# cs4247/music-transcription

Hardware: AMD Instinct MI355X
Metric: 30 s audio chunks/sec (mel+CNNRNN forward) (higher is better)
Workload: dtype f16; 1 GPU; CNNRNNModel inference, batch=32x30 s synthetic 16 kHz audio, mel+CNN-RNN HIP path (BASELINE.json configs[1]); batch_per_gpu=32, frames=938, coscheduled_batches_per_forward=4, streams_per_gpu=4, batches_in_flight=16, parallelism=dp1 (independent chunks)

## Files before the change

include/mt_hip.h:

```cpp
#ifndef MT_HIP_H
#define MT_HIP_H

#include <stddef.h>
#include <stdint.h>

#ifdef __cplusplus
extern "C" {
#endif

#define MT_OK            0
#define MT_EINVAL       -1
#define MT_EWORKSPACE   -2
#define MT_EHIP         -3
#define MT_EUNSUPPORTED -4

#define MT_DT_BF16 0
#define MT_DT_F16  1
#define MT_GX_F16  0x10

#define MT_N_FFT 2048
#define MT_N_PITCH 88

typedef void* mt_stream_t;

// ... 72 lines not shown
                              int B, int T, int N, int Hprev, mt_stream_t stream);
int    mt_gemm_f32acc_dt(const void* A, int lda, const void* W, int ldw, const float* bias,
                         float* C, int ldc, int M, int N, int K, int dt, mt_stream_t stream);
int    mt_gemm_lstm_gx_dt(const void* X, int ldx, const void* W_ih, int ldw, const float* bias, float* gx,
                          int B, int T, int H, int K, int dt, mt_stream_t stream);
int    mt_gemm_logits_dt(const void* X, int ldx, const void* W, int ldw, const float* bias, float* logits,
                         int B, int T, int N, int K, int dt, mt_stream_t stream);
#define MT_GEMM_SCHED_BYTES 64
size_t mt_gemm_sched_bytes(void);
int    mt_gemm_lstm_gx_sched(const void* X, int ldx, const void* W_ih, int ldw, const float* bias, float* gx,
                             int B, int T, int H, int K, int dt, void* sched, mt_stream_t stream);
int    mt_gemm_lstm_gx_from_hx_sched(const float* hx_prev, const void* W_ih, int ldw, const float* bias, float* gx,
                                     int B, int T, int H, int Hprev, int gx_f16, void* sched, mt_stream_t stream);

size_t mt_lstm_gx_bytes(int B, int T, int H);
size_t mt_lstm_hx_bytes(int B, int T, int H);
size_t mt_lstm_sync_bytes(int B, int H);
int    mt_lstm_bidir_fwd(const float* gx, const float* w_hh, float* hx, void* sync_ws, size_t sync_bytes,
                         int B, int T, int H, mt_stream_t stream);
int    mt_lstm_bidir_fwd_xproj(const float* hx_prev, const float* w_ihx, const float* bias, const float* w_hh, float* hx,
                               void* sync_ws, size_t sync_bytes, int B, int T, int H, mt_stream_t stream);
int    mt_lstm_bidir_fwd_ex(const float* gx, const float* w_hh, float* hx, void* sync_ws, size_t sync_bytes,
                            int B, int T, int H, int flags, mt_stream_t stream);
int    mt_persistent_cus_in_flight(mt_stream_t stream);
int    mt_lstm_relayout_bf16(const float* hx, void* X, int ldx, int B, int T, int H, mt_stream_t stream);
int    mt_lstm_unpack_f32(const float* hx, float* y, int B, int T, int H, mt_stream_t stream);

#define MT_MAX_LSTM_LAYERS 8
typedef struct {
    int n_mels;
    int hidden;
    int layers;
    int operand_dtype;
    const float* conv1_w;
    const float* conv1_b;
    const void*  conv2_w;
    const float* conv2_b;
    const void*  w_ih[MT_MAX_LSTM_LAYERS];
    const float* b_gates[MT_MAX_LSTM_LAYERS];
    const float* w_hh[MT_MAX_LSTM_LAYERS];
    const void*  fc_w;
    const float* fc_b;
    const float* w_ihx[MT_MAX_LSTM_LAYERS];
} mt_cnnrnn_weights;

size_t mt_cnnrnn_workspace_bytes(const mt_cnnrnn_weights* w, int B, int T);
// ... 301 lines not shown
```

music-transcription_amd/_lib.py:

```python
from __future__ import annotations

import ctypes as C
import os

_HERE = os.path.dirname(os.path.abspath(__file__))
LIB_PATH = os.path.join(_HERE, "libmt_hip.so")
MAX_LSTM_LAYERS = 8
N_PITCH = 88
DT_BF16, DT_F16 = 0, 1
GX_F16 = 0x10


class MtError(RuntimeError):
    pass


def build(verbose: bool = False) -> str:
    import subprocess
    r = subprocess.run(["make", "-C", os.path.join(_HERE, "csrc"), "-j8"], capture_output=True, text=True)
    if verbose or r.returncode != 0:
        print(r.stdout[-4000:], r.stderr[-4000:])
    if r.returncode != 0:
        raise MtError("building libmt_hip.so failed")
    return LIB_PATH
# ... 63 lines not shown
    "mt_conv_cl_dt": (i32, [vp, vp, vp, vp, vp] + [i32] * 12 + [vp]),
    "mt_gemm_batched_f32_dt": (i32, [vp, i32, ll, ll, vp, i32, ll, ll, vp, vp, i32, ll, ll, i32, i32, i32, i32, i32, i32, vp]),
    "mt_gemm_batched_h16out_dt": (i32, [vp, i32, ll, ll, vp, i32, ll, ll, vp, vp, i32, ll, ll, i32, i32, i32, i32, i32, i32, i32, vp]),
    "mt_lstm_relayout_dt": (i32, [vp, vp, i32, vp, i32, i32, i32, i32, i32, i32, i32, vp]),
    "mt_attn_softmax_clamped_dt": (i32, [vp, i32, vp, i32, i32, ll, C.c_float, C.c_float, i32, vp]),
    "mt_layernorm_residual_dt": (i32, [vp, i32, vp, i32, vp, vp, vp, i32, ll, i32, C.c_float, i32, vp]),
    "mt_gemm_lstm_gx_from_hx": (i32, [vp, vp, i32, vp, vp, i32, i32, i32, i32, vp]),
    "mt_gemm_lstm_gx_from_hx_ex": (i32, [vp, vp, i32, vp, vp, i32, i32, i32, i32, i32, vp]),
    "mt_gemm_logits_from_hx": (i32, [vp, vp, i32, vp, vp, i32, i32, i32, i32, vp]),
    "mt_gemm_bf16_f32acc": (i32, [vp, i32, vp, i32, vp, vp, i32, i32, i32, i32, vp]),
    "mt_gemm_lstm_gx": (i32, [vp, i32, vp, i32, vp, vp, i32, i32, i32, i32, vp]),
    "mt_gemm_sched_bytes": (sz, []),
    "mt_gemm_lstm_gx_sched": (i32, [vp, i32, vp, i32, vp, vp, i32, i32, i32, i32, i32, vp, vp]),
    "mt_gemm_lstm_gx_from_hx_sched": (i32, [vp, vp, i32, vp, vp, i32, i32, i32, i32, i32, vp, vp]),
    "mt_gemm_lstm_dh": (i32, [vp, i32, vp, i32, vp, i32, i32, i32, i32, i32, C.c_float, C.c_uint, C.c_uint, vp]),
    "mt_gemm_logits": (i32, [vp, i32, vp, i32, vp, vp, i32, i32, i32, i32, vp]),
    "mt_lstm_gx_bytes": (sz, [i32, i32, i32]),
    "mt_lstm_hx_bytes": (sz, [i32, i32, i32]),
    "mt_lstm_sync_bytes": (sz, [i32, i32]),
    "mt_lstm_bidir_fwd": (i32, [vp, vp, vp, vp, sz, i32, i32, i32, vp]),
    "mt_lstm_bidir_fwd_xproj": (i32, [vp, vp, vp, vp, vp, vp, sz, i32, i32, i32, vp]),
    "mt_lstm_bidir_fwd_ex": (i32, [vp, vp, vp, vp, sz, i32, i32, i32, i32, vp]),
    "mt_persistent_cus_in_flight": (i32, [vp]),
    "mt_lstm_relayout_bf16": (i32, [vp, vp, i32, i32, i32, i32, vp]),
    "mt_lstm_unpack_f32": (i32, [vp, vp, i32, i32, i32, vp]),
    "mt_conv_cl_bf16": (i32, [vp, vp, vp, vp, vp] + [i32] * 11 + [vp]),
    "mt_gemm_batched_f32": (i32, [vp, i32, ll, ll, vp, i32, ll, ll, vp, vp, i32, ll, ll, i32, i32, i32, i32, i32, vp]),
    "mt_gemm_batched_bf16out": (i32, [vp, i32, ll, ll, vp, i32, ll, ll, vp, vp, i32, ll, ll, i32, i32, i32, i32, i32, i32, vp]),
    "mt_lstm_relayout_ex": (i32, [vp, vp, i32, vp, i32, i32, i32, i32, i32, i32, vp]),
    "mt_attn_softmax_clamped": (i32, [vp, i32, vp, i32, i32, ll, C.c_float, C.c_float, vp]),
    "mt_attn_transpose_v": (i32, [vp, i32, i32, vp, i32, i32, i32, i32, i32, vp]),
    "mt_attn_fused_clamped": (i32, [vp, i32, i32, vp, i32, i32, i32, i32, i32, C.c_float, C.c_float, vp, i32, i32, vp]),
    "mt_layernorm_residual": (i32, [vp, i32, vp, i32, vp, vp, vp, i32, ll, i32, C.c_float, vp]),
    "mt_cnnrnn_large_workspace_bytes": (sz, [C.POINTER(CnnRnnLargeWeights), i32, i32]),
    "mt_cnnrnn_large_status_offset": (sz, [C.POINTER(CnnRnnLargeWeights), i32, i32, i32]),
    "mt_cnnrnn_large_forward": (i32, [C.POINTER(CnnRnnLargeWeights), vp, vp, i32, i32, vp, vp, sz, vp]),
    "mt_cnnrnn_large_forward_ex": (i32, [C.POINTER(CnnRnnLargeWeights), vp, vp, i32, i32, vp, vp, sz, vp, vp, vp, vp]),
    "mt_cnnrnn_large_num_stages": (i32, [i32]),
    "mt_cnnrnn_large_forward_ev": (i32, [C.POINTER(CnnRnnLargeWeights), vp, vp, i32, i32, vp, vp, sz, C.POINTER(vp), i32, vp]),
    "mt_adam_workspace_bytes": (sz, []),
    "mt_adam_clip_step": (i32, [vp, vp, vp, vp, ll] + [C.c_float] * 6 + [i32, vp, vp, sz, vp]),
    "mt_adam_clip_step_ex": (i32, [vp, vp, vp, vp, ll] + [C.c_float] * 6 + [i32, C.c_float, vp, i32, vp, vp, sz, vp]),
    "mt_adam_clip_step_ema": (i32, [vp, vp, vp, vp, vp, ll] + [C.c_float] * 6 + [i32, C.c_float, vp, i32, C.c_float, vp, vp, sz, vp]),
    "mt_swap_f32": (i32, [vp, vp, ll, vp]),
    "mt_bce_workspace_bytes": (sz, []),
    "mt_bce_masked_fwd_bwd": (i32, [vp, vp, vp, C.c_longlong, C.c_float, i32, vp, vp, vp, sz, i32, i32, i32, vp]),
# ... 109 lines not shown
```

music-transcription_amd/csrc/lstm.hip:

```cpp
#include "lstm_handoff.h"
#include <stdlib.h>

namespace mt {

struct LstmArgs {
    const float* gx;
    const float* w_hh;
    float* hx;
    unsigned* status;
    int B, T, H;
    int g0;
    int ngl;
    float* gates_out;
    float* cx;
    const float* w_ihx;
    const float* bias;
    const float* hx_prev;
    int sleep_first, sleep_retry;
};

__device__ __forceinline__ float sigmoidf_(float x) { return __builtin_amdgcn_rcpf(1.0f + __expf(-x)); }
__device__ __forceinline__ float tanhf_(float x) { return fmaf(2.0f, __builtin_amdgcn_rcpf(1.0f + __expf(-2.0f * x)), -1.0f); }
constexpr unsigned H_POISON = 0xFFFFFFFFu;
constexpr int PAYLOAD_POLL_SLEEP = 10;
constexpr int PAYLOAD_POLL_SLEEP_BUSY = 18;
constexpr int PAYLOAD_POLL_SLEEP_TRAIN = 12;

#ifdef MT_LSTM_DIAG
__device__ unsigned long long mt_lstm_diag[1024][8];
#define DIAG_STAMP(i) do { if (tid == 0) { const long long n_ = __builtin_amdgcn_s_memrealtime(); dg[i] += n_ - tl; tl = n_; } } while (0)
#else
#define DIAG_STAMP(i) do { } while (0)
#endif

typedef __attribute__((__vector_size__(4 * sizeof(int)))) int i32x4_t;
__device__ __forceinline__ i32x4_t raw_rsrc(const void* p, unsigned bytes) {
    const unsigned long long a = (unsigned long long)p;
    i32x4_t r;
    r[0] = __builtin_amdgcn_readfirstlane((int)(unsigned)a);
    r[1] = __builtin_amdgcn_readfirstlane((int)((unsigned)(a >> 32) & 0xffffu));
    r[2] = __builtin_amdgcn_readfirstlane((int)bytes);
    r[3] = 0x00020000;
    return r;
}
template <int OFF> __device__ __forceinline__ void asm_load_b128_sc1(u32x4& dst, int voff, i32x4_t rsrc) {
    asm volatile("buffer_load_dwordx4 %0, %1, %2, 0 offen offset:%3 sc1" : "=v"(dst) : "v"(voff), "s"(rsrc), "n"(OFF));
}
template <int NKSW, int I = 0> __device__ __forceinline__ void asm_gather_sc1(u32x4 (&hq)[NKSW], int voff, i32x4_t rsrc) {
    if constexpr (I < NKSW) {
        asm_load_b128_sc1<(I & 3) * 1024>(hq[I], voff + (I >> 2) * 4096, rsrc);
        asm_gather_sc1<NKSW, I + 1>(hq, voff, rsrc);
    }
}
__device__ __forceinline__ unsigned spin_clock() {
    return (unsigned)__builtin_amdgcn_readfirstlane((int)(unsigned)__builtin_amdgcn_s_memrealtime()) | 1u;
}
template <int N> __device__ __forceinline__ void vm_wait() { asm volatile("s_waitcnt vmcnt(%0)" :: "n"(N)); }
__device__ __forceinline__ void vm_settle(u32x4& v) { asm volatile("" : "+v"(v)); }

template <int NKSW, bool TRAIN = false, bool XP = false, int NG = 1, bool G16 = false>
__global__ __launch_bounds__(XP ? 256 : 320, XP ? 1 : (NKSW > 8 ? 2 : 4)) void lstm_rec_kernel(LstmArgs a) {
    __shared__ __attribute__((aligned(16))) float red[4][64][20];
    __shared__ __attribute__((aligned(16))) f16_t hs[32][8];
    constexpr int GX_RING = XP ? 1 : 6;
    constexpr int GX_DMA = G16 ? 2 : 4;
    __shared__ __attribute__((aligned(16))) float gring[GX_RING][XP ? 4 : (G16 ? 512 : 1024)];
    __shared__ int abort_s;
    const int tid = threadIdx.x, wv = __builtin_amdgcn_readfirstlane(tid >> 6), lane = tid & 63;
    const int H = a.H, T = a.T, nkb = H >> 3, nks = H >> 4;
    const int kb = blockIdx.x, d = blockIdx.y, gbase = blockIdx.z * NG + a.g0;
    const int ngh = min(NG, a.g0 + a.ngl - gbase);
    const int b = lane & 31, hh = lane >> 5;

    if (!XP && wv == 4) {
        typedef __attribute__((address_space(1))) void gvoid_t;
        typedef __attribute__((address_space(3))) void lvoid_t;
        const size_t gd_blocks_l = (size_t)T * 2 * nkb;
        const int nslots = T * ngh;
        int is = 0, ig = 0;
        auto request = [&](int n) {
            const int tn = d ? (T - 1 - is) : is;
            const size_t blk = (size_t)(gbase + ig) * gd_blocks_l + ((size_t)tn * 2 + d) * nkb + kb;
            const char* src = (const char*)a.gx + blk * (G16 ? 2048 : 4096) + lane * 16;
            char* dst = (char*)&gring[n % GX_RING][0];
#pragma unroll
            for (int qq = 0; qq < GX_DMA; ++qq) __builtin_amdgcn_global_load_lds((gvoid_t*)(src + qq * 1024), (lvoid_t*)(dst + qq * 1024), 16, 0, 0);
            if (++ig == ngh) { ig = 0; ++is; }
        };
        for (int n = 0; n < GX_RING - 1 && n < nslots; ++n) request(n);
        if (GX_RING - 1 <= nslots) asm volatile("s_waitcnt vmcnt(%0)" :: "n"(GX_DMA * (GX_RING - 2)) : "memory");
        else asm volatile("s_waitcnt vmcnt(0)" ::: "memory");
        __builtin_amdgcn_s_barrier();
        for (int n = 0; n < nslots; ++n) {
// ... 222 lines not shown
        }
#ifdef MT_LSTM_DIAG
        asm volatile("" :: "v"(hval));
#endif
        DIAG_STAMP(4);
        hs[b][jl] = (f16_t)hval;
        DIAG_STAMP(5);
        __syncthreads();
        if (wv == 0 && lane < 32) {
            const u32x4 piece = *(const u32x4*)(&hs[b][0]);
            const int hoff = ((t * 2 + d) * nkb) * 512 + (kb >> 1) * 1024 + ((kb & 1) * 32 + b) * 16;
            __builtin_amdgcn_raw_buffer_store_b128(piece, hrsrc, hoff, 0, 16 );
        }
        DIAG_STAMP(6);
      }
    }
    if (NG > 1) vm_wait<0>();
#ifdef MT_LSTM_DIAG
    if (tid == 0) {
        const int wg = (blockIdx.z * gridDim.y + blockIdx.y) * gridDim.x + blockIdx.x;
        for (int i = 0; i < 8; ++i) mt_lstm_diag[wg & 1023][i] = dg[i];
    }
#endif
}

template <int NK, bool TRAIN, bool G16>
__global__ __launch_bounds__(320, 4) void lstm_rec16_kernel(LstmArgs a) {
    __shared__ __attribute__((aligned(16))) float red[4][2][64][4];
    __shared__ __attribute__((aligned(16))) f16_t hs[32][8];
    constexpr int GX_RING = 6;
    constexpr int GX_DMA = G16 ? 2 : 4;
    __shared__ __attribute__((aligned(16))) float gring[GX_RING][G16 ? 512 : 1024];
    __shared__ int abort_s;
    const int tid = threadIdx.x, wv = tid >> 6, lane = tid & 63;
    const int H = a.H, T = a.T, nkb = H >> 3, nks = H >> 4;
    const int kb = blockIdx.x, d = blockIdx.y, g = blockIdx.z + a.g0;
    const int Bg = min(16, a.B - g * 32);
    const size_t gd_blocks = (size_t)T * 2 * nkb;

    if (wv == 4) {
        typedef __attribute__((address_space(1))) void gvoid_t;
        typedef __attribute__((address_space(3))) void lvoid_t;
        int is = 0;
        auto request = [&](int n) {
            const int tn = d ? (T - 1 - is) : is;
            const size_t blk = (size_t)g * gd_blocks + ((size_t)tn * 2 + d) * nkb + kb;
// ... 162 lines not shown
                                                         pack_bf16x2((float)h8[4], (float)h8[5]), pack_bf16x2((float)h8[6], (float)h8[7]));
            } else {
                for (int j = 0; j < 8 && kb * 8 + j < Hv; ++j) X[m * ldx + c0 + j] = f32_to_h16<DT>((float)h8[j]);
            }
        }
        if (Y)
            for (int j = 0; j < 8 && kb * 8 + j < Hv; ++j) Y[m * ldy + c0 + j] = (float)h8[j];
    }
}

__global__ void lstm_unpack_kernel(const f16_t* __restrict__ hx, float* __restrict__ y, int B, int T, int H) {
    const int nkb = H >> 3;
    const size_t total = (size_t)T * B * 2 * H;
    for (size_t id = (size_t)blockIdx.x * blockDim.x + threadIdx.x; id < total; id += (size_t)gridDim.x * blockDim.x) {
        const int k = id % H;
        const int d = (id / H) & 1;
        const size_t bt = id / (2 * H);
        const int t = bt % T, b = bt / T, g = b >> 5, bl = b & 31;
        const f16_t* blk = hx + ((((size_t)g * T + t) * 2 + d) * nkb) * 256 + (size_t)(k >> 4) * 512;
        y[id] = (float)blk[(((k >> 3) & 1) * 32 + bl) * 8 + (k & 7)];
    }
}

template <int NKSW, bool G16>
static int launch_rec_plain(const LstmArgs& a, int ngroups, hipStream_t st) {
    const dim3 one_set(a.H >> 3, 2, 1);
    if constexpr (NKSW <= 8) {
        if (ngroups == 2) return persistent_launch(lstm_rec_kernel<NKSW, false, false, 2, G16>, one_set, 320, a, st, "mt_lstm_bidir_fwd");
        if (ngroups == 3) return persistent_launch(lstm_rec_kernel<NKSW, false, false, 3, G16>, one_set, 320, a, st, "mt_lstm_bidir_fwd");
        if (ngroups > 3) return persistent_launch(lstm_rec_kernel<NKSW, false, false, 4, G16>, dim3(a.H >> 3, 2, cdiv(ngroups, 4)), 320, a, st, "mt_lstm_bidir_fwd");
    }
    return persistent_launch(lstm_rec_kernel<NKSW, false, false, 1, G16>, dim3(a.H >> 3, 2, ngroups), 320, a, st, "mt_lstm_bidir_fwd");
}

template <int NKSW>
static int launch_rec(const LstmArgs& a, int ngroups, bool g16, hipStream_t st) {
    const dim3 per_group(a.H >> 3, 2, ngroups);
    if constexpr (NKSW <= 8) {
        static const bool c16 = !(getenv("MT_LSTM_C16") && atoi(getenv("MT_LSTM_C16")) == 0);
        constexpr int NK16 = (NKSW + 1) / 2;
        if (c16 && !a.w_ihx && a.B <= 16 && ngroups == 1) {
            if (a.cx) return persistent_launch(lstm_rec16_kernel<NK16, true, false>, per_group, 320, a, st, "mt_lstm_bidir_fwd_train");
            if (g16) return persistent_launch(lstm_rec16_kernel<NK16, false, true>, per_group, 320, a, st, "mt_lstm_bidir_fwd");
            return persistent_launch(lstm_rec16_kernel<NK16, false, false>, per_group, 320, a, st, "mt_lstm_bidir_fwd");
        }
        if (a.w_ihx) return persistent_launch(lstm_rec_kernel<NKSW, false, true>, per_group, 256, a, st, "mt_lstm_bidir_fwd_xproj");
    }
    if (a.cx) return persistent_launch(lstm_rec_kernel<NKSW, true, false>, per_group, 320, a, st, "mt_lstm_bidir_fwd_train");
    return g16 ? launch_rec_plain<NKSW, true>(a, ngroups, st) : launch_rec_plain<NKSW, false>(a, ngroups, st);
}

}

using namespace mt;

extern "C" size_t mt_lstm_gx_bytes(int B, int T, int H) { return (size_t)cdiv(B, 32) * T * 2 * (H >> 3) * 4096; }
extern "C" size_t mt_lstm_hx_bytes(int B, int T, int H) { return (size_t)cdiv(B, 32) * T * 2 * (H >> 3) * 512; }
extern "C" size_t mt_lstm_sync_bytes(int B, int H) { (void)B; (void)H; return 512; }

static int lstm_fwd_impl(const float* gx, const float* w_hh, float* hx, void* sync_ws, size_t sync_bytes,
                         int B, int T, int H, int flags, mt_stream_t stream, float* cx = nullptr,
                         const float* w_ihx = nullptr, const float* bias = nullptr, const float* hx_prev = nullptr) {
    MT_REQUIRE((gx || w_ihx) && w_hh && hx && sync_ws, MT_EINVAL, "mt_lstm_bidir_fwd: null pointer");
    MT_REQUIRE(B > 0 && T > 0 && H >= 16 && H % 16 == 0 && H <= 1024, MT_EUNSUPPORTED,
               "mt_lstm_bidir_fwd: hidden size %d unsupported (multiple of 16, <= 1024)", H);
    MT_REQUIRE(sync_bytes >= mt_lstm_sync_bytes(B, H), MT_EWORKSPACE, "mt_lstm_bidir_fwd: sync workspace too small");
    const int nkb = H >> 3, ng = cdiv(B, 32);
    const bool g16 = (flags & MT_GX_F16) != 0;
    MT_REQUIRE(!g16 || (!cx && !w_ihx), MT_EINVAL, "mt_lstm_bidir_fwd_ex: MT_GX_F16 is for plain inference launches only");
    MT_REQUIRE((size_t)T * 2 * nkb * 512 < ((size_t)1 << 31), MT_EUNSUPPORTED, "mt_lstm_bidir_fwd: T*H too large for one buffer descriptor");
    MT_REQUIRE(!cx || (size_t)T * 2 * nkb * 4096 < ((size_t)1 << 31), MT_EUNSUPPORTED, "mt_lstm_bidir_fwd_train: T*H too large for one buffer descriptor of the gates");
    MT_REQUIRE((((size_t)w_hh | (size_t)w_ihx) & 15) == 0, MT_EINVAL, "mt_lstm_bidir_fwd: weight matrices must be 16-byte aligned");
    hipStream_t st = (hipStream_t)stream;
    MT_CHECK_HIP(hipMemsetAsync(sync_ws, 0, mt_lstm_sync_bytes(B, H), st));
    MT_CHECK_HIP(hipMemsetAsync(hx, 0xFF, mt_lstm_hx_bytes(B, T, H), st));
    static const int env_first = getenv("MT_LSTM_POLL_FIRST") ? atoi(getenv("MT_LSTM_POLL_FIRST")) : -1;
    static const int env_retry = getenv("MT_LSTM_POLL_RETRY") ? atoi(getenv("MT_LSTM_POLL_RETRY")) : -1;
    LstmArgs a{gx, w_hh, hx, (unsigned*)sync_ws, B, T, H, 0, 0,
               cx ? const_cast<float*>(gx) : nullptr, cx, w_ihx, bias, hx_prev,
               env_first >= 0 ? env_first : (cx ? PAYLOAD_POLL_SLEEP_TRAIN : ((!w_ihx && mt_persistent_cus_in_flight(stream) > 0) ? PAYLOAD_POLL_SLEEP_BUSY : PAYLOAD_POLL_SLEEP)),
               env_retry >= 0 ? env_retry : 0};
    const int zmax = (256 / (2 * nkb)) > 0 ? (256 / (2 * nkb)) : 1;
    const int nksw = cdiv(nkb / 2, 4);
    const int per_launch = (cx || w_ihx || nksw > 8) ? zmax : 4 * zmax;
    for (int g0 = 0; g0 < ng; g0 += per_launch) {
        a.g0 = g0;
        const int n = (ng - g0) < per_launch ? (ng - g0) : per_launch;
        a.ngl = n;
        int rc;
        if (nksw <= 1) rc = launch_rec<1>(a, n, g16, st);
        else if (nksw <= 2) rc = launch_rec<2>(a, n, g16, st);
        else if (nksw <= 4) rc = launch_rec<4>(a, n, g16, st);
        else if (nksw <= 8) rc = launch_rec<8>(a, n, g16, st);
        else rc = launch_rec<16>(a, n, g16, st);
        if (rc != MT_OK) return rc;
    }
    return MT_OK;
}

extern "C" int mt_lstm_bidir_fwd(const float* gx, const float* w_hh, float* hx, void* sync_ws, size_t sync_bytes,
                                 int B, int T, int H, mt_stream_t stream) {
    return lstm_fwd_impl(gx, w_hh, hx, sync_ws, sync_bytes, B, T, H, 0, stream);
}

extern "C" int mt_lstm_bidir_fwd_xproj(const float* hx_prev, const float* w_ihx, const float* bias, const float* w_hh, float* hx,
                                       void* sync_ws, size_t sync_bytes, int B, int T, int H, mt_stream_t stream) {
    MT_REQUIRE(hx_prev && w_ihx && bias && hx_prev != hx, MT_EINVAL, "mt_lstm_bidir_fwd_xproj: bad arguments");
    MT_REQUIRE(H <= 512, MT_EUNSUPPORTED, "mt_lstm_bidir_fwd_xproj: H=%d > 512 (the W_ih slice lives in registers)", H);
    return lstm_fwd_impl(nullptr, w_hh, hx, sync_ws, sync_bytes, B, T, H, 0, stream, nullptr, w_ihx, bias, hx_prev);
}

extern "C" int mt_lstm_bidir_fwd_train(float* gx_inout, const float* w_hh, float* hx, float* cx, void* sync_ws, size_t sync_bytes,
                                       int B, int T, int H, mt_stream_t stream) {
    MT_REQUIRE(cx, MT_EINVAL, "mt_lstm_bidir_fwd_train: null cx");
    return lstm_fwd_impl(gx_inout, w_hh, hx, sync_ws, sync_bytes, B, T, H, 0, stream, cx);
}

extern "C" int mt_lstm_bidir_fwd_ex(const float* gx, const float* w_hh, float* hx, void* sync_ws, size_t sync_bytes,
                                    int B, int T, int H, int flags, mt_stream_t stream) {
    MT_REQUIRE(flags == 0 || flags == MT_GX_F16, MT_EINVAL, "mt_lstm_bidir_fwd_ex: flags must be 0 or MT_GX_F16 (gx is f16)");
    return lstm_fwd_impl(gx, w_hh, hx, sync_ws, sync_bytes, B, T, H, flags, stream);
}

extern "C" int mt_lstm_relayout_dt(const float* hx, void* X, int ldx, float* Y, int ldy, int col_off, int B, int T, int H, int Hv,
                                   int dt, mt_stream_t stream) {
    MT_REQUIRE(hx && (X || Y) && H % 16 == 0 && Hv > 0 && Hv <= H && col_off >= 0, MT_EINVAL, "mt_lstm_relayout_ex: bad arguments");
    MT_REQUIRE((!X || (ldx >= col_off + 2 * Hv && ldx % 8 == 0)) && (!Y || ldy >= col_off + 2 * Hv), MT_EINVAL, "mt_lstm_relayout_ex: bad leading dimension");
    MT_REQUIRE_DT(dt, "mt_lstm_relayout");
    const size_t total = (size_t)T * B * 2 * ((Hv + 7) >> 3);
    MT_REQUIRE(total < ((size_t)1 << 31), MT_EUNSUPPORTED, "mt_lstm_relayout: more than 2^31 pieces");
    const int blocks = (int)((total + 255) / 256 < 4096 ? (total + 255) / 256 : 4096);
    const Div3 dv = make_div3((Hv + 7) >> 3, 2);
    unsigned mB, sB;
    div_magic((unsigned)B, &mB, &sB);
    if (dt == MT_DT_F16)
        hipLaunchKernelGGL(lstm_relayout_kernel<MT_DT_F16>, dim3(blocks), dim3(256), 0, (hipStream_t)stream, (const f16_t*)hx, (bf16_t*)X, ldx, Y, ldy,
                           col_off, B, T, H, Hv, dv, mB, sB);
    else
        hipLaunchKernelGGL(lstm_relayout_kernel<MT_DT_BF16>, dim3(blocks), dim3(256), 0, (hipStream_t)stream, (const f16_t*)hx, (bf16_t*)X, ldx, Y, ldy,
                           col_off, B, T, H, Hv, dv, mB, sB);
    MT_CHECK_LAUNCH();
    return MT_OK;
}
extern "C" int mt_lstm_relayout_ex(const float* hx, void* X, int ldx, float* Y, int ldy, int col_off, int B, int T, int H, int Hv,
                                   mt_stream_t stream) {
// ... 23 lines not shown
```

music-transcription_amd/csrc/lstm_handoff.h:

```cpp
#pragma once
#include "mt_common.h"

namespace mt {

constexpr int LSTM_SPIN_LIMIT_TICKS = 200000000;
constexpr int OOB_OFF = 0x7FFFFF00;
typedef __attribute__((__vector_size__(4 * sizeof(unsigned)))) unsigned u32x4;

__device__ __forceinline__ void sleep64(int n) {
    for (int i = 0; i < n; ++i) __builtin_amdgcn_s_sleep(1);
}

int persistent_admit(const void* kernel, int block, size_t smem, int nwg, hipStream_t st, const char* who);
int persistent_mark(hipStream_t st);
int persistent_cancel(hipStream_t st);

template <typename Args>
static int persistent_launch(void (*kernel)(Args), dim3 grid, int nthreads, const Args& a, hipStream_t st, const char* who,
                             const char* file = __builtin_FILE(), int line = __builtin_LINE()) {
    int rc = persistent_admit((const void*)kernel, nthreads, 0, (int)(grid.x * grid.y * grid.z), st, who);
    if (rc != MT_OK) return rc;
    hipLaunchKernelGGL(kernel, grid, dim3(nthreads), 0, st, a);
    const hipError_t e = hipGetLastError();
    if (e != hipSuccess) {
        persistent_cancel(st);
        set_error("%s:%d: persistent launch -> %s", file, line, hipGetErrorString(e));
        return MT_EHIP;
    }
    return persistent_mark(st);
}

}
```

music-transcription_amd/csrc/model.hip:

```cpp
#include "mt_common.h"
#include <stdlib.h>

extern "C" {
int mt_conv1_bn_relu_pool_dt(const float*, const float*, const float*, const float*, void*, int, int, int, int, mt_stream_t);
int mt_conv2_bn_relu_pool_dt(const void*, const void*, const float*, void*, int, int, int, int, int, mt_stream_t);
int mt_conv12_bn_relu_pool_dt(const float*, const float*, const float*, const float*, const void*, const float*, void*, int, int, int, int, int, mt_stream_t);
int mt_gemm_lstm_gx_dt(const void*, int, const void*, int, const float*, float*, int, int, int, int, int, mt_stream_t);
int mt_gemm_logits_dt(const void*, int, const void*, int, const float*, float*, int, int, int, int, int, mt_stream_t);
int mt_lstm_bidir_fwd_ex(const float*, const float*, float*, void*, size_t, int, int, int, int, mt_stream_t);
int mt_lstm_relayout_dt(const float*, void*, int, float*, int, int, int, int, int, int, int, mt_stream_t);
int mt_gemm_lstm_gx_from_hx_ex(const float*, const void*, int, const float*, float*, int, int, int, int, int, mt_stream_t);
int mt_gemm_logits_from_hx(const float*, const void*, int, const float*, float*, int, int, int, int, mt_stream_t);
int mt_gemm_lstm_gx_sched(const void*, int, const void*, int, const float*, float*, int, int, int, int, int, void*, mt_stream_t);
int mt_gemm_lstm_gx_from_hx_sched(const float*, const void*, int, const float*, float*, int, int, int, int, int, void*, mt_stream_t);
int mt_lstm_bidir_fwd_xproj(const float*, const float*, const float*, const float*, float*, void*, size_t, int, int, int, mt_stream_t);
size_t mt_lstm_gx_bytes(int, int, int);
size_t mt_lstm_hx_bytes(int, int, int);
size_t mt_lstm_sync_bytes(int, int);
}

namespace mt {
struct CnnRnnPlan {
    int F1, Fo2, K0, K1, M, Mpad, Hp;
    size_t act1, x0, x1, gx, hx, hx2, sync, sync_stride, sched, total;
// ... 68 lines not shown
    MT_REQUIRE(B > 0 && T > 0, MT_EINVAL, "mt_cnnrnn_forward: bad dims B=%d T=%d", B, T);
    const CnnRnnPlan p = plan(w, B, T);
    MT_REQUIRE(workspace_bytes >= p.total, MT_EWORKSPACE, "mt_cnnrnn_forward: workspace %zu < %zu bytes", workspace_bytes, p.total);
    char* ws = (char*)workspace;
    const int H = p.Hp, Hv = w->hidden, dt = w->operand_dtype;
    hipStream_t st = (hipStream_t)stream;
    int ei = 0;
    if ((rc = rec(events, n_events, ei, st)) != MT_OK) return rc;
    if (mt_cnnrnn_conv_fused()) {
        if ((rc = rec(events, n_events, ei, st)) != MT_OK) return rc;
        if ((rc = mt_conv12_bn_relu_pool_dt(mel, chunk_max_power, w->conv1_w, w->conv1_b, w->conv2_w, w->conv2_b, ws + p.x0, p.K0, B, w->n_mels, T, dt,
                                            stream)) != MT_OK) return rc;
    } else {
        if ((rc = mt_conv1_bn_relu_pool_dt(mel, chunk_max_power, w->conv1_w, w->conv1_b, ws + p.act1, B, w->n_mels, T, dt, stream)) != MT_OK) return rc;
        if ((rc = rec(events, n_events, ei, st)) != MT_OK) return rc;
        if ((rc = mt_conv2_bn_relu_pool_dt(ws + p.act1, w->conv2_w, w->conv2_b, ws + p.x0, p.K0, B, p.F1, T, dt, stream)) != MT_OK) return rc;
    }
    if ((rc = rec(events, n_events, ei, st)) != MT_OK) return rc;
    if (p.K1 != 2 * Hv) MT_CHECK_HIP(hipMemsetAsync(ws + p.x1, 0, (size_t)p.Mpad * p.K1 * 2, (hipStream_t)stream));
    char* hcur = ws + p.hx;
    char* hnext = ws + p.hx2;
    const bool from_hx = dt == MT_DT_F16 && H == Hv && H % 64 == 0;
    const int gx16 = (dt == MT_DT_F16) ? MT_GX_F16 : 0;
    for (int l = 0; l < w->layers; ++l) {
        const bool last = l + 1 == w->layers;
        const bool fused = l > 0 && w->w_ihx[l] && H <= 512;
        if (fused) {
            if ((rc = rec(events, n_events, ei, st)) != MT_OK) return rc;
            if ((rc = mt_lstm_bidir_fwd_xproj((const float*)hcur, w->w_ihx[l], w->b_gates[l], w->w_hh[l], (float*)hnext,
                                              ws + p.sync + p.sync_stride * l, p.sync_stride, B, T, H, stream)) != MT_OK) return rc;
            char* tmp = hcur; hcur = hnext; hnext = tmp;
        } else {
            const int K = l == 0 ? p.K0 : p.K1;
            if (l > 0 && from_hx) {
                if ((rc = mt_gemm_lstm_gx_from_hx_sched((const float*)hcur, w->w_ih[l], K, w->b_gates[l], (float*)(ws + p.gx), B, T, H, H, gx16,
                                                        ws + p.sched + (size_t)MT_GEMM_SCHED_BYTES * l, stream)) != MT_OK) return rc;
                char* tmp = hcur; hcur = hnext; hnext = tmp;
            } else {
                const void* X = l == 0 ? ws + p.x0 : ws + p.x1;
                if ((rc = mt_gemm_lstm_gx_sched(X, K, w->w_ih[l], K, w->b_gates[l], (float*)(ws + p.gx), B, T, H, K, dt | gx16,
                                                ws + p.sched + (size_t)MT_GEMM_SCHED_BYTES * l, stream)) != MT_OK) return rc;
            }
            if ((rc = rec(events, n_events, ei, st)) != MT_OK) return rc;
            if ((rc = mt_lstm_bidir_fwd_ex((const float*)(ws + p.gx), w->w_hh[l], (float*)hcur, ws + p.sync + p.sync_stride * l,
                                           p.sync_stride, B, T, H, gx16, stream)) != MT_OK) return rc;
        }
        if ((rc = rec(events, n_events, ei, st)) != MT_OK) return rc;
        const bool next_fused = !last && w->w_ihx[l + 1] && H <= 512;
        if (!next_fused && !from_hx)
            if ((rc = mt_lstm_relayout_dt((const float*)hcur, ws + p.x1, p.K1, nullptr, 0, 0, B, T, H, Hv, dt, stream)) != MT_OK) return rc;
        if ((rc = rec(events, n_events, ei, st)) != MT_OK) return rc;
    }
    if (from_hx) {
        if ((rc = mt_gemm_logits_from_hx((const float*)hcur, w->fc_w, p.K1, w->fc_b, logits, B, T, MT_N_PITCH, H, stream)) != MT_OK) return rc;
    } else {
        if ((rc = mt_gemm_logits_dt(ws + p.x1, p.K1, w->fc_w, p.K1, w->fc_b, logits, B, T, MT_N_PITCH, p.K1, dt, stream)) != MT_OK) return rc;
    }
    return rec(events, n_events, ei, st);
}

extern "C" int mt_cnnrnn_forward(const mt_cnnrnn_weights* w, const float* mel, const float* chunk_max_power, int B, int T,
                                 float* logits, void* workspace, size_t workspace_bytes, mt_stream_t stream) {
    return mt_cnnrnn_forward_ex(w, mel, chunk_max_power, B, T, logits, workspace, workspace_bytes, nullptr, 0, stream);
}
```

music-transcription_amd/csrc/residency.hip:

```cpp
#include "mt_common.h"
#include <mutex>
#include <vector>

namespace mt {

struct PersistentEntry {
    hipStream_t st;
    hipEvent_t ev;
    double need;
    bool pending;
    int reserved;
    double rneed;
};
static std::mutex g_mu;
static std::vector<PersistentEntry> g_tab[16];
static int g_ncu[16];

int persistent_admit(const void* kernel, int block, size_t smem, int nwg, hipStream_t st, const char* who) {
    int dev = 0;
    MT_CHECK_HIP(hipGetDevice(&dev));
    MT_REQUIRE(dev >= 0 && dev < 16, MT_EUNSUPPORTED, "%s: device index %d", who, dev);
    int per_cu = 0;
    MT_CHECK_HIP(hipOccupancyMaxActiveBlocksPerMultiprocessor(&per_cu, kernel, block, smem));
    MT_REQUIRE(per_cu >= 1, MT_EUNSUPPORTED, "%s: the kernel does not fit a CU", who);
    std::lock_guard<std::mutex> lock(g_mu);
    if (g_ncu[dev] == 0) MT_CHECK_HIP(hipDeviceGetAttribute(&g_ncu[dev], hipDeviceAttributeMultiprocessorCount, dev));
    const double need = (double)nwg / per_cu, cap = (double)g_ncu[dev];
    MT_REQUIRE(need <= cap, MT_EUNSUPPORTED, "%s: %d workgroups at %d per CU cannot be resident on %d CUs", who, nwg, per_cu, g_ncu[dev]);
    double others = 0.0;
    PersistentEntry* mine = nullptr;
    for (auto& e : g_tab[dev]) {
        if (e.pending && hipEventQuery(e.ev) == hipSuccess) { e.pending = false; e.need = 0.0; }
        if (e.st == st) mine = &e;
        else others += (e.pending ? e.need : 0.0) > e.rneed ? (e.pending ? e.need : 0.0) : e.rneed;
    }
    (void)hipGetLastError();
    if (others + need > cap + 1e-9) {
        set_error("%s: %.0f CUs for this persistent launch + %.0f CUs held by persistent launches pending on other streams > %d CUs: "
                  "they could not all be resident and would stall on each other (fewer forwards in flight per GPU)",
                  who, need, others, g_ncu[dev]);
        return MT_EUNSUPPORTED;
    }
    if (!mine) {
        PersistentEntry e{st, nullptr, 0.0, false, 0, 0.0};
        MT_CHECK_HIP(hipEventCreateWithFlags(&e.ev, hipEventDisableTiming));
        g_tab[dev].push_back(e);
        mine = &g_tab[dev].back();
    }
    mine->reserved += 1;
    mine->rneed = mine->rneed > need ? mine->rneed : need;
    return MT_OK;
}

static PersistentEntry* find_entry(int dev, hipStream_t st) {
    for (auto& e : g_tab[dev])
        if (e.st == st) return &e;
    return nullptr;
}

int persistent_cancel(hipStream_t st) {
    int dev = 0;
    if (hipGetDevice(&dev) != hipSuccess || dev < 0 || dev >= 16) return MT_EHIP;
    std::lock_guard<std::mutex> lock(g_mu);
    if (PersistentEntry* e = find_entry(dev, st)) {
        if (e->reserved > 0 && --e->reserved == 0) e->rneed = 0.0;
    }
    return MT_OK;
}

int persistent_mark(hipStream_t st) {
    int dev = 0;
    MT_CHECK_HIP(hipGetDevice(&dev));
    std::lock_guard<std::mutex> lock(g_mu);
    if (PersistentEntry* e = find_entry(dev, st)) {
        const double was = e->pending ? e->need : 0.0;
        MT_CHECK_HIP(hipEventRecord(e->ev, st));
        e->need = was > e->rneed ? was : e->rneed;
        e->pending = true;
        if (e->reserved > 0 && --e->reserved == 0) e->rneed = 0.0;
    }
    return MT_OK;
}

}

extern "C" int mt_persistent_cus_in_flight(mt_stream_t stream) {
    int dev = 0;
    if (hipGetDevice(&dev) != hipSuccess || dev < 0 || dev >= 16) return MT_EHIP;
    std::lock_guard<std::mutex> lock(mt::g_mu);
    double others = 0.0;
    for (auto& e : mt::g_tab[dev]) {
        if (e.pending && hipEventQuery(e.ev) == hipSuccess) { e.pending = false; e.need = 0.0; }
        if (e.st != (hipStream_t)stream) others += (e.pending ? e.need : 0.0) > e.rneed ? (e.pending ? e.need : 0.0) : e.rneed;
    }
    (void)hipGetLastError();
    return (int)(others + 0.5);
}
```

Before: 8818 chunks/s.

## Add adaptive wide LSTM recurrence that splits groups across two workgroup sets when GPU idle

Adds a lstm_wide_kernel that launches two sets of recurrence workgroups and decides at runtime, via a device-wide running counter, whether to split the batch groups across both sets (wide) or use only one (narrow). The wide split is chosen when no other LSTM recurrence is running, so per-set work per timestep shrinks and latency falls when the GPU is otherwise underused. Residency admission gains surplus accounting so the extra workgroups count against CU capacity, and the model marks chained LSTM layers as held/kept so the running counter spans the whole stack. Costs: doubled grid with idle early-exit workgroups, extra claim/spin handshake, and more CU reservation, which could reduce how many forwards can run concurrently.

```diff
diff --git a/include/mt_hip.h b/include/mt_hip.h
--- a/include/mt_hip.h
+++ b/include/mt_hip.h
@@ -118,6 +118,11 @@
                                void* sync_ws, size_t sync_bytes, int B, int T, int H, mt_stream_t stream);
 int    mt_lstm_bidir_fwd_ex(const float* gx, const float* w_hh, float* hx, void* sync_ws, size_t sync_bytes,
                             int B, int T, int H, int flags, mt_stream_t stream);
+#define MT_LSTM_HELD 0x100
+#define MT_LSTM_KEEP 0x200
+int    mt_lstm_set_width_mode(int mode);
+size_t mt_lstm_width_offset(void);
+int    mt_persistent_fits(const double* need, const double* surplus, int n, int ncu);
 int    mt_persistent_cus_in_flight(mt_stream_t stream);
 int    mt_lstm_relayout_bf16(const float* hx, void* X, int ldx, int B, int T, int H, mt_stream_t stream);
 int    mt_lstm_unpack_f32(const float* hx, float* y, int B, int T, int H, mt_stream_t stream);
diff --git a/music-transcription_amd/_lib.py b/music-transcription_amd/_lib.py
--- a/music-transcription_amd/_lib.py
+++ b/music-transcription_amd/_lib.py
@@ -109,6 +109,9 @@
     "mt_lstm_bidir_fwd_xproj": (i32, [vp, vp, vp, vp, vp, vp, sz, i32, i32, i32, vp]),
     "mt_lstm_bidir_fwd_ex": (i32, [vp, vp, vp, vp, sz, i32, i32, i32, i32, vp]),
     "mt_persistent_cus_in_flight": (i32, [vp]),
+    "mt_persistent_fits": (i32, [C.POINTER(C.c_double), C.POINTER(C.c_double), i32, i32]),
+    "mt_lstm_set_width_mode": (i32, [i32]),
+    "mt_lstm_width_offset": (sz, []),
     "mt_lstm_relayout_bf16": (i32, [vp, vp, i32, i32, i32, i32, vp]),
     "mt_lstm_unpack_f32": (i32, [vp, vp, i32, i32, i32, vp]),
     "mt_conv_cl_bf16": (i32, [vp, vp, vp, vp, vp] + [i32] * 11 + [vp]),
diff --git a/music-transcription_amd/csrc/lstm.hip b/music-transcription_amd/csrc/lstm.hip
--- a/music-transcription_amd/csrc/lstm.hip
+++ b/music-transcription_amd/csrc/lstm.hip
@@ -1,5 +1,6 @@
 #include "lstm_handoff.h"
 #include <stdlib.h>
+#include <atomic>
 
 namespace mt {
 
@@ -17,6 +18,7 @@
     const float* bias;
     const float* hx_prev;
     int sleep_first, sleep_retry;
+    int hold, width, width_word;
 };
 
 __device__ __forceinline__ float sigmoidf_(float x) { return __builtin_amdgcn_rcpf(1.0f + __expf(-x)); }
@@ -58,17 +60,42 @@
 template <int N> __device__ __forceinline__ void vm_wait() { asm volatile("s_waitcnt vmcnt(%0)" :: "n"(N)); }
 __device__ __forceinline__ void vm_settle(u32x4& v) { asm volatile("" : "+v"(v)); }
 
+template <bool XP, bool G16>
+struct RecShared {
+    float red[4][64][20];
+    f16_t hs[32][8];
+    float gring[XP ? 1 : 6][XP ? 4 : (G16 ? 512 : 1024)];
+    int abort_s;
+};
+
+__device__ unsigned mt_lstm_running;
+constexpr int HOLD_BEGIN = 1, HOLD_END = 2;
+constexpr unsigned WIDTH_NARROW = 1u, WIDTH_WIDE = 2u;
+constexpr int SYNC_WIDTH_WORD = 32;
+
+template <int NKSW, bool TRAIN, bool XP, int NG, bool G16>
+__device__ __forceinline__ void lstm_rec_body(const LstmArgs& a, const int zidx, RecShared<XP, G16>& sh);
+
 template <int NKSW, bool TRAIN = false, bool XP = false, int NG = 1, bool G16 = false>
 __global__ __launch_bounds__(XP ? 256 : 320, XP ? 1 : (NKSW > 8 ? 2 : 4)) void lstm_rec_kernel(LstmArgs a) {
-    __shared__ __attribute__((aligned(16))) float red[4][64][20];
-    __shared__ __attribute__((aligned(16))) f16_t hs[32][8];
+    __shared__ __attribute__((aligned(16))) RecShared<XP, G16> sh;
+    const bool keeper = !TRAIN && !XP && (blockIdx.x | blockIdx.y | blockIdx.z) == 0 && threadIdx.x == 0;
+    if (keeper && (a.hold & HOLD_BEGIN)) __hip_atomic_fetch_add(&mt_lstm_running, 1u, __ATOMIC_RELAXED, __HIP_MEMORY_SCOPE_AGENT);
+    lstm_rec_body<NKSW, TRAIN, XP, NG, G16>(a, blockIdx.z, sh);
+    if (keeper && (a.hold & HOLD_END)) __hip_atomic_fetch_sub(&mt_lstm_running, 1u, __ATOMIC_RELAXED, __HIP_MEMORY_SCOPE_AGENT);
+}
+
+template <int NKSW, bool TRAIN, bool XP, int NG, bool G16>
+__device__ __forceinline__ void lstm_rec_body(const LstmArgs& a, const int zidx, RecShared<XP, G16>& sh) {
+    float (&red)[4][64][20] = sh.red;
+    f16_t (&hs)[32][8] = sh.hs;
     constexpr int GX_RING = XP ? 1 : 6;
     constexpr int GX_DMA = G16 ? 2 : 4;
-    __shared__ __attribute__((aligned(16))) float gring[GX_RING][XP ? 4 : (G16 ? 512 : 1024)];
-    __shared__ int abort_s;
+    float (&gring)[GX_RING][XP ? 4 : (G16 ? 512 : 1024)] = sh.gring;
+    int& abort_s = sh.abort_s;
     const int tid = threadIdx.x, wv = __builtin_amdgcn_readfirstlane(tid >> 6), lane = tid & 63;
     const int H = a.H, T = a.T, nkb = H >> 3, nks = H >> 4;
-    const int kb = blockIdx.x, d = blockIdx.y, gbase = blockIdx.z * NG + a.g0;
+    const int kb = blockIdx.x, d = blockIdx.y, gbase = zidx * NG + a.g0;
     const int ngh = min(NG, a.g0 + a.ngl - gbase);
     const int b = lane & 31, hh = lane >> 5;
 
@@ -337,6 +364,60 @@
         for (int i = 0; i < 8; ++i) mt_lstm_diag[wg & 1023][i] = dg[i];
     }
 #endif
+}
+
+template <int NKSW, int NG, bool G16>
+__global__ __launch_bounds__(320, 4) void lstm_wide_kernel(LstmArgs a) {
+    static_assert(NKSW <= 8 && NG >= 2 && NG <= 4, "the interleaved plain inference instances");
+    __shared__ __attribute__((aligned(16))) RecShared<false, G16> sh;
+    __shared__ unsigned width_s;
+    unsigned* const claim = a.status + a.width_word;
+    if (threadIdx.x == 0) {
+        unsigned dec = 0;
+        if (__hip_atomic_exchange(claim, 1u, __ATOMIC_RELAXED, __HIP_MEMORY_SCOPE_AGENT) == 0u) {
+            const unsigned others = (a.hold & HOLD_BEGIN) ? __hip_atomic_fetch_add(&mt_lstm_running, 1u, __ATOMIC_RELAXED, __HIP_MEMORY_SCOPE_AGENT)
+                                                          : __hip_atomic_load(&mt_lstm_running, __ATOMIC_RELAXED, __HIP_MEMORY_SCOPE_AGENT) - 1u;
+            dec = a.width == 3 ? WIDTH_WIDE : (a.width == 2 ? WIDTH_NARROW : (others == 0u ? WIDTH_WIDE : WIDTH_NARROW));
+            __hip_atomic_store(claim + 1, dec, __ATOMIC_RELEASE, __HIP_MEMORY_SCOPE_AGENT);
+        } else {
+            unsigned t1 = 0;
+            for (unsigned it = 0;; ++it) {
+                dec = __hip_atomic_load(claim + 1, __ATOMIC_ACQUIRE, __HIP_MEMORY_SCOPE_AGENT);
+                if (dec != 0u) break;
+                sleep64(2);
+                if ((it & 63u) == 63u && __hip_atomic_load(a.status, __ATOMIC_RELAXED, __HIP_MEMORY_SCOPE_AGENT) != 0u) break;
+                if ((it & 255u) == 255u) {
+                    const unsigned now = spin_clock();
+                    if (t1 == 0) t1 = now;
+                    else if (now - t1 > (unsigned)LSTM_SPIN_LIMIT_TICKS) {
+                        __hip_atomic_store(a.status, 0x40000000u, __ATOMIC_RELAXED, __HIP_MEMORY_SCOPE_AGENT);
+                        break;
+                    }
+                }
+            }
+        }
+        width_s = dec;
+    }
+    __syncthreads();
+    const unsigned dec = (unsigned)__builtin_amdgcn_readfirstlane((int)width_s);
+    if (dec == 0u) return;
+    const int set = blockIdx.z;
+    constexpr int N0 = (NG + 1) / 2, N1 = NG - N0;
+    if (dec == WIDTH_NARROW) {
+        if (set == 0) lstm_rec_body<NKSW, false, false, NG, G16>(a, 0, sh);
+    } else {
+        LstmArgs h = a;
+        if (set == 0) {
+            h.ngl = N0;
+            lstm_rec_body<NKSW, false, false, N0, G16>(h, 0, sh);
+        } else {
+            h.g0 = a.g0 + N0;
+            h.ngl = N1;
+            lstm_rec_body<NKSW, false, false, N1, G16>(h, 0, sh);
+        }
+    }
+    if ((a.hold & HOLD_END) && (blockIdx.x | blockIdx.y | blockIdx.z) == 0 && threadIdx.x == 0)
+        __hip_atomic_fetch_sub(&mt_lstm_running, 1u, __ATOMIC_RELAXED, __HIP_MEMORY_SCOPE_AGENT);
 }
 
 template <int NK, bool TRAIN, bool G16>
@@ -545,22 +626,44 @@
     }
 }
 
+template <int NKSW, int NG, bool G16>
+static int launch_rec_sets(LstmArgs a, hipStream_t st) {
+    const int nwg = 2 * (a.H >> 3);
+    int wide_ok = 0;
+    const int rc = persistent_admit((const void*)lstm_wide_kernel<NKSW, NG, G16>, 320, 0, nwg, st, "mt_lstm_bidir_fwd", nwg, a.width == 3, &wide_ok);
+    if (rc != MT_OK) return rc;
+    if (wide_ok) return persistent_fire(lstm_wide_kernel<NKSW, NG, G16>, dim3(a.H >> 3, 2, 2), 320, a, st);
+    a.width = 0;
+    return persistent_fire(lstm_rec_kernel<NKSW, false, false, NG, G16>, dim3(a.H >> 3, 2, 1), 320, a, st);
+}
+
 template <int NKSW, bool G16>
 static int launch_rec_plain(const LstmArgs& a, int ngroups, hipStream_t st) {
     const dim3 one_set(a.H >> 3, 2, 1);
     if constexpr (NKSW <= 8) {
+        if (a.width != 0) {
+            if (ngroups == 2) return launch_rec_sets<NKSW, 2, G16>(a, st);
+            if (ngroups == 3) return launch_rec_sets<NKSW, 3, G16>(a, st);
+            if (ngroups == 4) return launch_rec_sets<NKSW, 4, G16>(a, st);
+        }
         if (ngroups == 2) return persistent_launch(lstm_rec_kernel<NKSW, false, false, 2, G16>, one_set, 320, a, st, "mt_lstm_bidir_fwd");
         if (ngroups == 3) return persistent_launch(lstm_rec_kernel<NKSW, false, false, 3, G16>, one_set, 320, a, st, "mt_lstm_bidir_fwd");
         if (ngroups > 3) return persistent_launch(lstm_rec_kernel<NKSW, false, false, 4, G16>, dim3(a.H >> 3, 2, cdiv(ngroups, 4)), 320, a, st, "mt_lstm_bidir_fwd");
     }
     return persistent_launch(lstm_rec_kernel<NKSW, false, false, 1, G16>, dim3(a.H >> 3, 2, ngroups), 320, a, st, "mt_lstm_bidir_fwd");
 }
+
+static bool lstm_c16() {
+    static const bool c16 = !(getenv("MT_LSTM_C16") && atoi(getenv("MT_LSTM_C16")) == 0);
+    return c16;
+}
+static std::atomic<int> g_width_mode{0};
 
 template <int NKSW>
 static int launch_rec(const LstmArgs& a, int ngroups, bool g16, hipStream_t st) {
     const dim3 per_group(a.H >> 3, 2, ngroups);
     if constexpr (NKSW <= 8) {
-        static const bool c16 = !(getenv("MT_LSTM_C16") && atoi(getenv("MT_LSTM_C16")) == 0);
+        const bool c16 = lstm_c16();
         constexpr int NK16 = (NKSW + 1) / 2;
         if (c16 && !a.w_ihx && a.B <= 16 && ngroups == 1) {
             if (a.cx) return persistent_launch(lstm_rec16_kernel<NK16, true, false>, per_group, 320, a, st, "mt_lstm_bidir_fwd_train");
@@ -602,14 +705,22 @@
     LstmArgs a{gx, w_hh, hx, (unsigned*)sync_ws, B, T, H, 0, 0,
                cx ? const_cast<float*>(gx) : nullptr, cx, w_ihx, bias, hx_prev,
                env_first >= 0 ? env_first : (cx ? PAYLOAD_POLL_SLEEP_TRAIN : ((!w_ihx && mt_persistent_cus_in_flight(stream) > 0) ? PAYLOAD_POLL_SLEEP_BUSY : PAYLOAD_POLL_SLEEP)),
-               env_retry >= 0 ? env_retry : 0};
+               env_retry >= 0 ? env_retry : 0, 0, 0, 0};
     const int zmax = (256 / (2 * nkb)) > 0 ? (256 / (2 * nkb)) : 1;
     const int nksw = cdiv(nkb / 2, 4);
     const int per_launch = (cx || w_ihx || nksw > 8) ? zmax : 4 * zmax;
-    for (int g0 = 0; g0 < ng; g0 += per_launch) {
+    const bool plain = !cx && !w_ihx && !(nksw <= 8 && B <= 16 && lstm_c16());
+    const int width_mode = g_width_mode.load(std::memory_order_relaxed);
+    int li = 0;
+    for (int g0 = 0; g0 < ng; g0 += per_launch, ++li) {
         a.g0 = g0;
         const int n = (ng - g0) < per_launch ? (ng - g0) : per_launch;
         a.ngl = n;
+        if (plain) {
+            a.hold = ((g0 == 0 && !(flags & MT_LSTM_HELD)) ? HOLD_BEGIN : 0) | ((g0 + per_launch >= ng && !(flags & MT_LSTM_KEEP)) ? HOLD_END : 0);
+            a.width_word = SYNC_WIDTH_WORD + 2 * li;
+            a.width = (nksw <= 8 && n >= 2 && n <= 4 && (size_t)(a.width_word + 2) * 4 <= mt_lstm_sync_bytes(B, H)) ? width_mode + 1 : 0;
+        }
         int rc;
         if (nksw <= 1) rc = launch_rec<1>(a, n, g16, st);
         else if (nksw <= 2) rc = launch_rec<2>(a, n, g16, st);
@@ -641,9 +752,16 @@
 
 extern "C" int mt_lstm_bidir_fwd_ex(const float* gx, const float* w_hh, float* hx, void* sync_ws, size_t sync_bytes,
                                     int B, int T, int H, int flags, mt_stream_t stream) {
-    MT_REQUIRE(flags == 0 || flags == MT_GX_F16, MT_EINVAL, "mt_lstm_bidir_fwd_ex: flags must be 0 or MT_GX_F16 (gx is f16)");
+    MT_REQUIRE((flags & ~(MT_GX_F16 | MT_LSTM_HELD | MT_LSTM_KEEP)) == 0, MT_EINVAL, "mt_lstm_bidir_fwd_ex: flags: MT_GX_F16 (gx is f16), MT_LSTM_HELD, MT_LSTM_KEEP");
     return lstm_fwd_impl(gx, w_hh, hx, sync_ws, sync_bytes, B, T, H, flags, stream);
 }
+
+extern "C" int mt_lstm_set_width_mode(int mode) {
+    MT_REQUIRE(mode >= 0 && mode <= 2, MT_EINVAL, "mt_lstm_set_width_mode: mode %d (0 auto, 1 narrow, 2 wide)", mode);
+    g_width_mode.store(mode, std::memory_order_relaxed);
+    return MT_OK;
+}
+extern "C" size_t mt_lstm_width_offset(void) { return (size_t)(SYNC_WIDTH_WORD + 1) * 4; }
 
 extern "C" int mt_lstm_relayout_dt(const float* hx, void* X, int ldx, float* Y, int ldy, int col_off, int B, int T, int H, int Hv,
                                    int dt, mt_stream_t stream) {
diff --git a/music-transcription_amd/csrc/lstm_handoff.h b/music-transcription_amd/csrc/lstm_handoff.h
--- a/music-transcription_amd/csrc/lstm_handoff.h
+++ b/music-transcription_amd/csrc/lstm_handoff.h
@@ -11,15 +11,14 @@
     for (int i = 0; i < n; ++i) __builtin_amdgcn_s_sleep(1);
 }
 
-int persistent_admit(const void* kernel, int block, size_t smem, int nwg, hipStream_t st, const char* who);
+int persistent_admit(const void* kernel, int block, size_t smem, int nwg, hipStream_t st, const char* who, int surplus_wg = 0, bool forced = false,
+                     int* wide_ok = nullptr);
 int persistent_mark(hipStream_t st);
 int persistent_cancel(hipStream_t st);
 
 template <typename Args>
-static int persistent_launch(void (*kernel)(Args), dim3 grid, int nthreads, const Args& a, hipStream_t st, const char* who,
-                             const char* file = __builtin_FILE(), int line = __builtin_LINE()) {
-    int rc = persistent_admit((const void*)kernel, nthreads, 0, (int)(grid.x * grid.y * grid.z), st, who);
-    if (rc != MT_OK) return rc;
+static int persistent_fire(void (*kernel)(Args), dim3 grid, int nthreads, const Args& a, hipStream_t st,
+                           const char* file = __builtin_FILE(), int line = __builtin_LINE()) {
     hipLaunchKernelGGL(kernel, grid, dim3(nthreads), 0, st, a);
     const hipError_t e = hipGetLastError();
     if (e != hipSuccess) {
@@ -30,4 +29,12 @@
     return persistent_mark(st);
 }
 
+template <typename Args>
+static int persistent_launch(void (*kernel)(Args), dim3 grid, int nthreads, const Args& a, hipStream_t st, const char* who,
+                             const char* file = __builtin_FILE(), int line = __builtin_LINE()) {
+    int rc = persistent_admit((const void*)kernel, nthreads, 0, (int)(grid.x * grid.y * grid.z), st, who);
+    if (rc != MT_OK) return rc;
+    return persistent_fire(kernel, grid, nthreads, a, st, file, line);
 }
+
+}
diff --git a/music-transcription_amd/csrc/model.hip b/music-transcription_amd/csrc/model.hip
--- a/music-transcription_amd/csrc/model.hip
+++ b/music-transcription_amd/csrc/model.hip
@@ -114,8 +114,11 @@
     char* hnext = ws + p.hx2;
     const bool from_hx = dt == MT_DT_F16 && H == Hv && H % 64 == 0;
     const int gx16 = (dt == MT_DT_F16) ? MT_GX_F16 : 0;
+    bool chain = true;
+    for (int l = 1; l < w->layers; ++l) chain = chain && !(w->w_ihx[l] && H <= 512);
     for (int l = 0; l < w->layers; ++l) {
         const bool last = l + 1 == w->layers;
+        const int hold = chain ? ((l > 0 ? MT_LSTM_HELD : 0) | (!last ? MT_LSTM_KEEP : 0)) : 0;
         const bool fused = l > 0 && w->w_ihx[l] && H <= 512;
         if (fused) {
             if ((rc = rec(events, n_events, ei, st)) != MT_OK) return rc;
@@ -135,7 +138,7 @@
             }
             if ((rc = rec(events, n_events, ei, st)) != MT_OK) return rc;
             if ((rc = mt_lstm_bidir_fwd_ex((const float*)(ws + p.gx), w->w_hh[l], (float*)hcur, ws + p.sync + p.sync_stride * l,
-                                           p.sync_stride, B, T, H, gx16, stream)) != MT_OK) return rc;
+                                           p.sync_stride, B, T, H, gx16 | hold, stream)) != MT_OK) return rc;
         }
         if ((rc = rec(events, n_events, ei, st)) != MT_OK) return rc;
         const bool next_fused = !last && w->w_ihx[l + 1] && H <= 512;
diff --git a/music-transcription_amd/csrc/residency.hip b/music-transcription_amd/csrc/residency.hip
--- a/music-transcription_amd/csrc/residency.hip
+++ b/music-transcription_amd/csrc/residency.hip
@@ -1,6 +1,15 @@
 #include "mt_common.h"
 #include <mutex>
 #include <vector>
+
+extern "C" int mt_persistent_fits(const double* need, const double* surplus, int n, int ncu) {
+    double sum = 0.0, mx = 0.0;
+    for (int i = 0; i < n; ++i) {
+        sum += need[i];
+        if (surplus && surplus[i] > mx) mx = surplus[i];
+    }
+    return sum + mx <= (double)ncu + 1e-9 ? 1 : 0;
+}
 
 namespace mt {
 
@@ -11,12 +20,18 @@
     bool pending;
     int reserved;
     double rneed;
+    double extra;
+    double rextra;
 };
 static std::mutex g_mu;
 static std::vector<PersistentEntry> g_tab[16];
 static int g_ncu[16];
 
-int persistent_admit(const void* kernel, int block, size_t smem, int nwg, hipStream_t st, const char* who) {
+static inline double dmax(double a, double b) { return a > b ? a : b; }
+static double held(const PersistentEntry& e) { return dmax(e.pending ? e.need : 0.0, e.rneed); }
+static double held_extra(const PersistentEntry& e) { return dmax(e.pending ? e.extra : 0.0, e.rextra); }
+
+int persistent_admit(const void* kernel, int block, size_t smem, int nwg, hipStream_t st, const char* who, int surplus_wg, bool forced, int* wide_ok) {
     int dev = 0;
     MT_CHECK_HIP(hipGetDevice(&dev));
     MT_REQUIRE(dev >= 0 && dev < 16, MT_EUNSUPPORTED, "%s: device index %d", who, dev);
@@ -25,30 +40,42 @@
     MT_REQUIRE(per_cu >= 1, MT_EUNSUPPORTED, "%s: the kernel does not fit a CU", who);
     std::lock_guard<std::mutex> lock(g_mu);
     if (g_ncu[dev] == 0) MT_CHECK_HIP(hipDeviceGetAttribute(&g_ncu[dev], hipDeviceAttributeMultiprocessorCount, dev));
-    const double need = (double)nwg / per_cu, cap = (double)g_ncu[dev];
+    double need = (double)nwg / per_cu, extra = (double)surplus_wg / per_cu;
+    const double cap = (double)g_ncu[dev];
     MT_REQUIRE(need <= cap, MT_EUNSUPPORTED, "%s: %d workgroups at %d per CU cannot be resident on %d CUs", who, nwg, per_cu, g_ncu[dev]);
-    double others = 0.0;
+    double others = 0.0, others_extra = 0.0;
     PersistentEntry* mine = nullptr;
     for (auto& e : g_tab[dev]) {
-        if (e.pending && hipEventQuery(e.ev) == hipSuccess) { e.pending = false; e.need = 0.0; }
+        if (e.pending && hipEventQuery(e.ev) == hipSuccess) { e.pending = false; e.need = 0.0; e.extra = 0.0; }
         if (e.st == st) mine = &e;
-        else others += (e.pending ? e.need : 0.0) > e.rneed ? (e.pending ? e.need : 0.0) : e.rneed;
+        else { others += held(e); others_extra = dmax(others_extra, held_extra(e)); }
     }
     (void)hipGetLastError();
-    if (others + need > cap + 1e-9) {
+    if (wide_ok) *wide_ok = 0;
+    if (surplus_wg > 0) {
+        const double n[2] = {others, need + (forced ? extra : 0.0)}, x[2] = {others_extra, forced ? 0.0 : extra};
+        if (wide_ok && mt_persistent_fits(n, x, 2, g_ncu[dev])) {
+            *wide_ok = 1;
+            if (forced) { need += extra; extra = 0.0; }
+        } else {
+            extra = 0.0;
+        }
+    }
+    if (others + need + dmax(others_extra, extra) > cap + 1e-9) {
         set_error("%s: %.0f CUs for this persistent launch + %.0f CUs held by persistent launches pending on other streams > %d CUs: "
                   "they could not all be resident and would stall on each other (fewer forwards in flight per GPU)",
                   who, need, others, g_ncu[dev]);
         return MT_EUNSUPPORTED;
     }
     if (!mine) {
-        PersistentEntry e{st, nullptr, 0.0, false, 0, 0.0};
+        PersistentEntry e{st, nullptr, 0.0, false, 0, 0.0, 0.0, 0.0};
         MT_CHECK_HIP(hipEventCreateWithFlags(&e.ev, hipEventDisableTiming));
         g_tab[dev].push_back(e);
         mine = &g_tab[dev].back();
     }
     mine->reserved += 1;
     mine->rneed = mine->rneed > need ? mine->rneed : need;
+    mine->rextra = dmax(mine->rextra, extra);
     return MT_OK;
 }
 
@@ -63,7 +90,7 @@
     if (hipGetDevice(&dev) != hipSuccess || dev < 0 || dev >= 16) return MT_EHIP;
     std::lock_guard<std::mutex> lock(g_mu);
     if (PersistentEntry* e = find_entry(dev, st)) {
-        if (e->reserved > 0 && --e->reserved == 0) e->rneed = 0.0;
+        if (e->reserved > 0 && --e->reserved == 0) { e->rneed = 0.0; e->rextra = 0.0; }
     }
     return MT_OK;
 }
@@ -74,10 +101,12 @@
     std::lock_guard<std::mutex> lock(g_mu);
     if (PersistentEntry* e = find_entry(dev, st)) {
         const double was = e->pending ? e->need : 0.0;
+        const double wasx = e->pending ? e->extra : 0.0;
         MT_CHECK_HIP(hipEventRecord(e->ev, st));
         e->need = was > e->rneed ? was : e->rneed;
+        e->extra = dmax(wasx, e->rextra);
         e->pending = true;
-        if (e->reserved > 0 && --e->reserved == 0) e->rneed = 0.0;
+        if (e->reserved > 0 && --e->reserved == 0) { e->rneed = 0.0; e->rextra = 0.0; }
     }
     return MT_OK;
 }
@@ -90,8 +119,8 @@
     std::lock_guard<std::mutex> lock(mt::g_mu);
     double others = 0.0;
     for (auto& e : mt::g_tab[dev]) {
-        if (e.pending && hipEventQuery(e.ev) == hipSuccess) { e.pending = false; e.need = 0.0; }
-        if (e.st != (hipStream_t)stream) others += (e.pending ? e.need : 0.0) > e.rneed ? (e.pending ? e.need : 0.0) : e.rneed;
+        if (e.pending && hipEventQuery(e.ev) == hipSuccess) { e.pending = false; e.need = 0.0; e.extra = 0.0; }
+        if (e.st != (hipStream_t)stream) others += mt::held(e);
     }
     (void)hipGetLastError();
     return (int)(others + 0.5);
```

New measurement: 9045 chunks/s, median of 6. 2.6% higher.
